# cpockrandt/PhyloCSFpp

Measured on NVIDIA B200. Metric: MAF columns/sec (6 frames, coding+noncoding ECM), higher is better.
Workload: dtype tf32x3/f32

## Files before the change

phylocsfpp_b200/csrc/model_prep.hpp:

```cpp
#pragma once

#include <cmath>
#include <cstdint>
#include <cstring>
#include <string>
#include <vector>

namespace pcsf {

constexpr int NS = 64;

constexpr int SMALL_TREE_MAX_LEAVES = 128;
constexpr int BLS_MAX_WORDS = 8;

struct LeafSet {
    uint64_t w[BLS_MAX_WORDS] = {};
    LeafSet operator|(const LeafSet &o) const { LeafSet r; for (int i = 0; i < BLS_MAX_WORDS; ++i) r.w[i] = w[i] | o.w[i]; return r; }
    LeafSet operator&(const LeafSet &o) const { LeafSet r; for (int i = 0; i < BLS_MAX_WORDS; ++i) r.w[i] = w[i] & o.w[i]; return r; }
    LeafSet operator~() const { LeafSet r; for (int i = 0; i < BLS_MAX_WORDS; ++i) r.w[i] = ~w[i]; return r; }
    bool any() const { uint64_t x = 0; for (int i = 0; i < BLS_MAX_WORDS; ++i) x |= w[i]; return x != 0; }
    int count() const { int c = 0; for (int i = 0; i < BLS_MAX_WORDS; ++i) c += __builtin_popcountll(w[i]); return c; }
    int first() const { for (int i = 0; i < BLS_MAX_WORDS; ++i) if (w[i]) return 64 * i + __builtin_ctzll(w[i]); return -1; }
    void set(int l) { w[l >> 6] |= 1ull << (l & 63); }
    static LeafSet all(int nl) { LeafSet r; for (int l = 0; l < nl; ++l) r.set(l); return r; }
    uint64_t bits(int shift, int nbits) const {
        const int i = shift >> 6, o = shift & 63;
        uint64_t v = w[i] >> o;
        if (o && i + 1 < BLS_MAX_WORDS) v |= w[i + 1] << (64 - o);
        return v & ((1ull << nbits) - 1);
    }
};

enum : int32_t { OP_GATHER_SET = 1, OP_GATHER_MUL = 2, OP_PUSH = 3, OP_POP_MUL = 4, OP_GEMM = 5, OP_END = 6 };
inline int32_t mk_op(int code, int arg) { return (code << 16) | (arg & 0xffff); }

struct BlsNode {
    double bl;
    LeafSet self;
    LeafSet left;
    int32_t is_leaf;
};

struct BlsInner {
    double bl;
    double left_bl, right_bl;
    LeafSet self, left;
    int32_t flags;
    int32_t tab_off;
};
inline int bls_table_shift(int32_t flags) { return ((flags >> 8) & 0xff) | ((flags >> 16) & 0xff00); }
inline int32_t bls_table_flags(int shift, int nbits) { return 4 | ((shift & 0xff) << 8) | (nbits << 16) | ((shift >> 8) << 24); }

template <int NW>
struct BlsInnerDev {
    double bl;
    double left_bl, right_bl;
    uint64_t self[NW], left[NW];
    int32_t flags;
    int32_t tab_off;
};
template <int NW>
inline std::vector<BlsInnerDev<NW>> bls_device_program(const std::vector<BlsInner> &prog) {
    std::vector<BlsInnerDev<NW>> out(prog.size());
    for (size_t k = 0; k < prog.size(); ++k) {
        const BlsInner &e = prog[k];
        BlsInnerDev<NW> &d = out[k];
        d.bl = e.bl; d.left_bl = e.left_bl; d.right_bl = e.right_bl;
        for (int i = 0; i < NW; ++i) { d.self[i] = e.self.w[i]; d.left[i] = e.left.w[i]; }
        d.flags = e.flags; d.tab_off = e.tab_off;
    }
    return out;
}

struct EcmHost {
    double lambda[NS], SR[NS * NS], SRinv[NS * NS], pi[NS], logpi[NS];
    std::vector<double> P;
    std::vector<double> pstream;
    std::vector<double> leafPT;
    std::vector<float> pstream_tc5;
    std::vector<double> cherry_P;
};

struct Tc5Src {
    uint32_t row_base;
    uint8_t l1, l2;
    uint8_t cherry;
    uint8_t pad;
};

struct ModelHost {
    int nl = 0, n = 0;
    std::vector<int16_t> child1, child2;
    std::vector<float> bl;
    std::vector<double> bl64;
    EcmHost ecm[2];
    std::vector<int32_t> program;
    std::vector<int> gemm_edges;
    int max_stack = 0;
    std::vector<uint32_t> tc5_steps;
    std::vector<int> tc5_edges;
    std::vector<int> tc5_leaf_order;
    std::vector<int> tc5_cherries;
    std::vector<uint16_t> tc5_cherry_leaves;
    std::vector<Tc5Src> tc5_srcs;
    uint32_t tc5_rows = 0;
    uint32_t tc5_start = 0;
    int tc5_max_stack = 0;
    std::vector<BlsNode> bls_prog;
    std::vector<BlsInner> bls_inner;
    std::vector<BlsInner> bls_short;
    std::vector<double> bls_tables;
    int bls_short_depth = 0;
    int bls_depth = 0;
    double bls_all = 0.0;
};

inline void build_q(const double *S, const double *f, double *Q) {
    double scale = 0.0;
    for (int i = 0; i < NS; ++i) {
        double rowsum = 0.0;
        for (int j = 0; j < NS; ++j) {
            const double v = S[i * NS + j] * f[j];
            Q[i * NS + j] = v;
            rowsum -= v;
        }
        Q[i * NS + i] = rowsum;
        scale -= rowsum * f[i];
    }
    for (int i = 0; i < NS * NS; ++i) Q[i] /= scale;
}

inline void jacobi64(std::vector<double> &A, std::vector<double> &V, double *w) {
    for (int i = 0; i < NS; ++i)
        for (int j = 0; j < NS; ++j) V[i * NS + j] = (i == j);
    for (int sweep = 0; sweep < 128; ++sweep) {
        double off = 0.0;
        for (int p = 0; p < NS; ++p)
            for (int q = p + 1; q < NS; ++q) off += A[p * NS + q] * A[p * NS + q];
        if (off < 1e-300) break;
        for (int p = 0; p + 1 < NS; ++p)
            for (int q = p + 1; q < NS; ++q) {
                const double apq = A[p * NS + q];
                if (std::fabs(apq) < 1e-310) continue;
                const double theta = (A[q * NS + q] - A[p * NS + p]) / (2.0 * apq);
                const double t = std::copysign(1.0, theta) / (std::fabs(theta) + std::sqrt(theta * theta + 1.0));
                const double c = 1.0 / std::sqrt(t * t + 1.0), s = t * c;
                for (int k = 0; k < NS; ++k) {
                    const double x = A[k * NS + p], y = A[k * NS + q];
                    A[k * NS + p] = c * x - s * y;
                    A[k * NS + q] = s * x + c * y;
                }
                for (int k = 0; k < NS; ++k) {
                    const double x = A[p * NS + k], y = A[q * NS + k];
                    A[p * NS + k] = c * x - s * y;
                    A[q * NS + k] = s * x + c * y;
                }
                for (int k = 0; k < NS; ++k) {
                    const double x = V[k * NS + p], y = V[k * NS + q];
                    V[k * NS + p] = c * x - s * y;
                    V[k * NS + q] = s * x + c * y;
                }
            }
    }
    for (int i = 0; i < NS; ++i) w[i] = A[i * NS + i];
}

inline bool eigen_and_prior(const double *Q, const double *f, EcmHost &e, std::string &err) {
    double sq[NS];
    for (int i = 0; i < NS; ++i) {
        if (!(f[i] > 0.0)) { err = "codon frequencies must be strictly positive"; return false; }
        sq[i] = std::sqrt(f[i]);
    }
    std::vector<double> A(NS * NS), U(NS * NS);
    for (int i = 0; i < NS; ++i)
        for (int j = 0; j < NS; ++j) A[i * NS + j] = sq[i] * Q[i * NS + j] / sq[j];
    for (int i = 0; i < NS; ++i)
        for (int j = i + 1; j < NS; ++j) A[i * NS + j] = A[j * NS + i] = 0.5 * (A[i * NS + j] + A[j * NS + i]);
    jacobi64(A, U, e.lambda);
    for (int i = 0; i < NS; ++i)
        for (int k = 0; k < NS; ++k) {
            e.SR[i * NS + k] = U[i * NS + k] / sq[i];
            e.SRinv[k * NS + i] = U[i * NS + k] * sq[i];
        }
    int kmin = 0;
    double best = std::fabs(e.lambda[0]);
    for (int k = 1; k < NS; ++k)
        if (std::fabs(e.lambda[k]) < best) { best = std::fabs(e.lambda[k]); kmin = k; }
    double mass = 0.0;
    for (int j = 0; j < NS; ++j) mass += e.SRinv[kmin * NS + j];
    for (int j = 0; j < NS; ++j) {
        e.pi[j] = e.SRinv[kmin * NS + j] / mass;
        e.logpi[j] = std::log(e.pi[j]);
    }
    return true;
}

inline double branch_time(float bl, double rho) { return (double)(float)((double)bl * rho); }

inline int pmatrix(const EcmHost &e, double t, double *P) {
    double ex[NS];
    std::vector<double> B(NS * NS);
    for (int k = 0; k < NS; ++k) ex[k] = std::exp(e.lambda[k] * t);
    for (int k = 0; k < NS; ++k)
        for (int j = 0; j < NS; ++j) B[k * NS + j] = e.SRinv[k * NS + j] * ex[k];
    for (int i = 0; i < NS; ++i) {
        double *row = P + i * NS;
        for (int j = 0; j < NS; ++j) row[j] = 0.0;
        for (int k = 0; k < NS; ++k) {
            const double a = e.SR[i * NS + k];
            for (int j = 0; j < NS; ++j) row[j] += a * B[k * NS + j];
        }
    }
    for (int i = 0; i < NS; ++i) {
        double total = 0.0, diag = 1.0;
        for (int j = 0; j < NS; ++j) {
            const double cell = P[i * NS + j];
            total += cell;
            if (cell < 0.0) {
                if (std::fabs(cell) > 1e-6) return 1;
                P[i * NS + j] = 0.0;
            }
            if (i != j) diag -= P[i * NS + j];
        }
        if (std::fabs(total - 1.0) > 1e-6) return 2;
        P[i * NS + i] = diag;
    }
    return 0;
}

inline void to_fragment_order(const double *P, double *tile) {
    for (int ks = 0; ks < 16; ++ks)
        for (int ntp = 0; ntp < 4; ++ntp)
            for (int lane = 0; lane < 32; ++lane)
                for (int e = 0; e < 2; ++e) {
                    const int a = 8 * (2 * ntp + e) + lane / 4;
                    const int b = 8 * (ks / 2) + 2 * (lane % 4) + (ks % 2);
                    tile[((ks * 4 + ntp) * 32 + lane) * 2 + e] = P[a * NS + b];
                }
}

// ... 384 lines not shown
```

phylocsfpp_b200/csrc/pcsf_capi.cu:

```cuda
#include "../../include/phylocsf_b200.h"

#include <cuda_runtime.h>

#include <algorithm>
#include <cmath>
#include <cstdio>
#include <cstdlib>
#include <cstring>
#include <limits>
#include <string>
#include <vector>

#include "kernels.cuh"
#include "mle.cuh"
#include "omega.cuh"
#include "prune_tc5.cuh"
#include "regions.cuh"
#include <nvtx3/nvToolsExt.h>

using namespace pcsf;

static thread_local std::string g_err;
static pcsf_status fail(pcsf_status st, const std::string &msg) { g_err = msg; return st; }

// ... 4 lines not shown
            return fail(PCSF_ERR_CUDA, std::string(#call) + ": " + cudaGetErrorString(e_));        \
    } while (0)

struct DevBuf {
    void *p = nullptr;
    size_t cap = 0;
    cudaError_t reserve(size_t bytes) {
        if (bytes <= cap) return cudaSuccess;
        if (p) cudaFree(p);
        p = nullptr; cap = 0;
        size_t want = bytes + bytes / 4;
        want = (want + ((size_t)2 << 20) - 1) & ~(((size_t)2 << 20) - 1);
        cudaError_t e = cudaMalloc(&p, want);
        if (e != cudaSuccess) { cudaGetLastError(); want = bytes; e = cudaMalloc(&p, want); }
        if (e == cudaSuccess) cap = want;
        return e;
    }
    void release() { if (p) cudaFree(p); p = nullptr; cap = 0; }
    template <class T> T *as() const { return reinterpret_cast<T *>(p); }
};

struct NvtxRange {
    explicit NvtxRange(const char *name) { nvtxRangePushA(name); }
    ~NvtxRange() { nvtxRangePop(); }
};

struct pcsf_model {
    int device = 0;
    int sm_count = 148;
    cudaStream_t own_stream = nullptr;
    cudaStream_t copy_stream = nullptr;
    cudaEvent_t ev_chunk = nullptr;
    double *h_plus = nullptr, *h_minus = nullptr, *h_bls = nullptr;
    uint32_t *h_pat = nullptr;
    const uint8_t *h_seqs = nullptr;
    int64_t h_ld = 0;
    cudaStream_t h2d_stream = nullptr;
    std::vector<cudaEvent_t> ev_h2d;
    ModelHost host;
    double *d_pstream[2] = {nullptr, nullptr}, *d_leafPT[2] = {nullptr, nullptr};
    double *d_pi[2] = {nullptr, nullptr}, *d_logpi[2] = {nullptr, nullptr};
    double *d_eig[2] = {nullptr, nullptr};
    float *d_pstream_tc5[2] = {nullptr, nullptr};
    float *d_rowtab_tc5[2] = {nullptr, nullptr};
    Tc5Src *d_tc5_srcs = nullptr;
    uint32_t *d_tc5_steps = nullptr;
    float *d_tc5_scratch = nullptr;
    size_t prune_tc5_smem = 0;
    int tc5_nstage = 2, tc5_nids = 1;
    MleStats msa_stats;
    uint8_t *h_msa = nullptr;
    size_t h_msa_cap = 0;
    DevBuf tc5_ids;
    int32_t *d_program = nullptr;
    void *d_bls_prog = nullptr;
    double *d_bls_tables = nullptr;
    float *d_bl = nullptr;
    int32_t *d_gemm_edges = nullptr;
    DevBuf codes, klo, khi, slot, flag, uniq, pidx, table, bsums, logz, anc, io_in, io_out, perwin, mle;
    DevBuf rg_units, rg_regions, rg_win;
    std::vector<pcsf_region> regions;
    int *d_bad = nullptr;
    uint32_t *d_nuniq = nullptr;
    int64_t chunk_cols = (int64_t)1 << 21;
    bool timing = false;
    uint32_t stagger_ns = 1000;
    pcsf_tracks_stats last{};
    int64_t last_nwin = 0;
    int launches = 0;
    int last_chunks = 0;
    int64_t codes_ld = 0;
    size_t prune_smem = 0;
    int prune_nwarp = 8;
    cudaEvent_t ev[8] = {};
};

static const int MAX_CHUNKS = 4096;

extern "C" const char *pcsf_last_error(void) { return g_err.c_str(); }
extern "C" int pcsf_abi_version(void) { return PCSF_ABI_VERSION; }

static pcsf_status upload(const void *src, size_t bytes, void **dst) {
    CK(cudaMalloc(dst, bytes ? bytes : 16));
    if (bytes) CK(cudaMemcpy(*dst, src, bytes, cudaMemcpyHostToDevice));
    return PCSF_OK;
}

extern "C" pcsf_status pcsf_model_create(const pcsf_model_desc *d, int device, pcsf_model **out) {
    if (!d || !out || d->nl < 2 || !d->child1 || !d->child2 || !d->branch_len || !d->branch_len_f64 || !d->ecm_c ||
        !d->freq_c || !d->ecm_nc || !d->freq_nc)
        return fail(PCSF_ERR_INVALID, "pcsf_model_create: null argument or fewer than 2 leaves");
    if (d->nl > PCSF_MAX_LEAVES)
        return fail(PCSF_ERR_UNSUPPORTED, "tree of " + std::to_string(d->nl) + " leaves: at most " + std::to_string(PCSF_MAX_LEAVES) +
                                              " leaves (PCSF_MAX_LEAVES) are supported");
    pcsf_model *m = new pcsf_model;
    struct Guard {
        pcsf_model *m;
        ~Guard() { if (m) pcsf_model_destroy(m); }
    } guard{m};
    const double *S[2] = {d->ecm_c, d->ecm_nc}, *f[2] = {d->freq_c, d->freq_nc};
    const std::string err = prepare_model(m->host, d->nl, d->child1, d->child2, d->branch_len, d->branch_len_f64, S, f);
    if (!err.empty()) {
        return fail(err.find("substition_matrix") != std::string::npos ? PCSF_ERR_NUMERIC : PCSF_ERR_INVALID, err);
    }
    int ndev = 0;
    if (cudaGetDeviceCount(&ndev) != cudaSuccess || ndev == 0 || device < 0 || device >= ndev) {
        guard.m = nullptr;
        delete m;
        return fail(PCSF_ERR_CUDA, "no CUDA device available (this library has no CPU fallback)");
    }
    m->device = device;
    if (const char *e = getenv("PCSF_STAGGER_NS")) m->stagger_ns = (uint32_t)atoi(e);
    CK(cudaSetDevice(device));
    CK(cudaDeviceGetAttribute(&m->sm_count, cudaDevAttrMultiProcessorCount, device));
    {
        uint8_t lut[256];
        memset(lut, 255, sizeof lut);
        lut['A'] = lut['a'] = 0; lut['C'] = lut['c'] = 1; lut['G'] = lut['g'] = 2; lut['T'] = lut['t'] = 3;
        lut['.'] = lut['-'] = lut['N'] = lut['n'] = 4;
        CK(cudaMemcpyToSymbol(c_dna_lut, lut, sizeof lut));
    }
    pcsf_status st;
    for (int w = 0; w < 2; ++w) {
        const EcmHost &e = m->host.ecm[w];
        if ((st = upload(e.pstream.data(), e.pstream.size() * 8, (void **)&m->d_pstream[w]))) return st;
        if ((st = upload(e.leafPT.data(), e.leafPT.size() * 8, (void **)&m->d_leafPT[w]))) return st;
        if ((st = upload(e.pstream_tc5.data(), e.pstream_tc5.size() * 4, (void **)&m->d_pstream_tc5[w]))) return st;
        if ((st = upload(e.pi, 64 * 8, (void **)&m->d_pi[w]))) return st;
        if ((st = upload(e.logpi, 64 * 8, (void **)&m->d_logpi[w]))) return st;
        std::vector<double> eig(64 + 2 * 4096);
        memcpy(eig.data(), e.lambda, 64 * 8);
        memcpy(eig.data() + 64, e.SR, 4096 * 8);
        memcpy(eig.data() + 64 + 4096, e.SRinv, 4096 * 8);
        if ((st = upload(eig.data(), eig.size() * 8, (void **)&m->d_eig[w]))) return st;
    }
    if ((st = upload(m->host.program.data(), m->host.program.size() * 4, (void **)&m->d_program))) return st;
    if (m->host.nl <= SMALL_TREE_MAX_LEAVES) {
        if ((st = upload(m->host.tc5_steps.data(), m->host.tc5_steps.size() * 4, (void **)&m->d_tc5_steps))) return st;
        CK(cudaMalloc(&m->d_tc5_scratch, (size_t)m->sm_count * 2 * std::max(1, m->host.tc5_max_stack) * T5_STACK_ENTRY_FLOATS * 4));
        const int ns = (int)m->host.tc5_srcs.size();
        if ((st = upload(m->host.tc5_srcs.data(), (size_t)ns * sizeof(Tc5Src), (void **)&m->d_tc5_srcs))) return st;
        for (int w = 0; w < 2; ++w) {
            double *d_cp = nullptr;
            if ((st = upload(m->host.ecm[w].cherry_P.data(), m->host.ecm[w].cherry_P.size() * 8, (void **)&d_cp))) return st;
            cudaError_t e = cudaMalloc(&m->d_rowtab_tc5[w], (size_t)m->host.tc5_rows * 64 * 4);
            if (e == cudaSuccess) {
                k_build_rows<<<dim3(65, ns), 64>>>(m->d_tc5_srcs, d_cp, m->d_leafPT[w], m->d_rowtab_tc5[w]);
                e = cudaGetLastError();
                if (e == cudaSuccess) e = cudaDeviceSynchronize();
            }
            cudaFree(d_cp);
            CK(e);
        }
        prune_tc5_pick_stages(m->host.nl, (int)m->host.tc5_steps.size(), (int)m->host.tc5_srcs.size(), &m->tc5_nstage, &m->tc5_nids);
        if (const char *e = getenv("PCSF_TC5_NSTAGE")) m->tc5_nstage = std::max(2, std::min(m->tc5_nstage, atoi(e)));
        if (const char *e = getenv("PCSF_TC5_NIDS")) m->tc5_nids = std::max(1, std::min(m->tc5_nids, atoi(e)));
        m->prune_tc5_smem = prune_tc5_smem_bytes(m->host.nl, (int)m->host.tc5_steps.size(), (int)m->host.tc5_srcs.size(), m->tc5_nstage, m->tc5_nids);
        if (m->prune_tc5_smem <= 227 * 1024)
            CK(cudaFuncSetAttribute(k_prune_tc5, cudaFuncAttributeMaxDynamicSharedMemorySize, (int)m->prune_tc5_smem));
        const std::vector<BlsInnerDev<2>> prog = bls_device_program<2>(m->host.bls_short);
        if ((st = upload(prog.data(), prog.size() * sizeof(prog[0]), &m->d_bls_prog))) return st;
    } else {
        const std::vector<BlsInnerDev<8>> prog = bls_device_program<8>(m->host.bls_short);
        if ((st = upload(prog.data(), prog.size() * sizeof(prog[0]), &m->d_bls_prog))) return st;
    }
    if ((st = upload(m->host.bls_tables.data(), std::max<size_t>(m->host.bls_tables.size(), 1) * sizeof(double), (void **)&m->d_bls_tables))) return st;
    if ((st = upload(m->host.bl.data(), m->host.bl.size() * 4, (void **)&m->d_bl))) return st;
    {
        std::vector<int32_t> ge(m->host.gemm_edges.begin(), m->host.gemm_edges.end());
        if ((st = upload(ge.data(), ge.size() * 4, (void **)&m->d_gemm_edges))) return st;
    }
    CK(cudaMalloc(&m->d_bad, sizeof(int)));
    CK(cudaMemset(m->d_bad, 0, sizeof(int)));
    if (!getenv("PCSF_LEGACY_STREAM")) {
        CK(cudaStreamCreateWithFlags(&m->own_stream, cudaStreamNonBlocking));
        CK(cudaStreamCreateWithFlags(&m->copy_stream, cudaStreamNonBlocking));
        CK(cudaStreamCreateWithFlags(&m->h2d_stream, cudaStreamNonBlocking));
        CK(cudaEventCreateWithFlags(&m->ev_chunk, cudaEventDisableTiming));
    }
    CK(cudaMalloc(&m->d_nuniq, sizeof(uint32_t) * MAX_CHUNKS));
    for (auto &e : m->ev) CK(cudaEventCreate(&e));
    m->prune_nwarp = PR_MAX_NWARP;
    if (const char *e = getenv("PCSF_PRUNE_NWARP")) m->prune_nwarp = std::max(1, std::min(PR_MAX_NWARP, atoi(e)));
    while (m->prune_nwarp > 4 &&
           prune_smem_bytes(m->host.nl, (int)m->host.program.size(), m->host.max_stack, m->prune_nwarp) > 227 * 1024)
        m->prune_nwarp -= 4;
    m->prune_smem = prune_smem_bytes(m->host.nl, (int)m->host.program.size(), m->host.max_stack, m->prune_nwarp);
    if (m->prune_smem > 227 * 1024) {
        return fail(PCSF_ERR_UNSUPPORTED, "tree needs more shared memory than one SM has (stack depth " +
                                              std::to_string(m->host.max_stack) + ")");
    }
    CK(cudaFuncSetAttribute(prune_kernel<false>(m->host.nl), cudaFuncAttributeMaxDynamicSharedMemorySize, (int)m->prune_smem));
    CK(cudaFuncSetAttribute(prune_kernel<true>(m->host.nl), cudaFuncAttributeMaxDynamicSharedMemorySize, (int)m->prune_smem));
    CK(cudaFuncSetAttribute(m->host.nl <= SMALL_TREE_MAX_LEAVES ? (const void *)k_bls<2> : (const void *)k_bls<8>,
                            cudaFuncAttributeMaxDynamicSharedMemorySize, std::max(1, m->host.bls_short_depth) * BLS_THREADS * BLS_COLS * 8));
    guard.m = nullptr;
    *out = m;
    return PCSF_OK;
}

extern "C" void pcsf_model_destroy(pcsf_model *m) {
    if (!m) return;
    cudaSetDevice(m->device);
    for (int w = 0; w < 2; ++w) {
        cudaFree(m->d_pstream[w]); cudaFree(m->d_leafPT[w]); cudaFree(m->d_rowtab_tc5[w]); cudaFree(m->d_pstream_tc5[w]); cudaFree(m->d_pi[w]); cudaFree(m->d_logpi[w]);
        cudaFree(m->d_eig[w]);
    }
    cudaFree(m->d_program); cudaFree(m->d_bls_prog); cudaFree(m->d_bls_tables); cudaFree(m->d_bl); cudaFree(m->d_gemm_edges);
    cudaFree(m->d_bad); cudaFree(m->d_nuniq); cudaFree(m->d_tc5_steps); cudaFree(m->d_tc5_scratch); cudaFree(m->d_tc5_srcs);
    if (m->h_msa) cudaFreeHost(m->h_msa);
    if (m->own_stream) cudaStreamDestroy(m->own_stream);
    if (m->copy_stream) cudaStreamDestroy(m->copy_stream);
    if (m->h2d_stream) cudaStreamDestroy(m->h2d_stream);
    for (cudaEvent_t e : m->ev_h2d) cudaEventDestroy(e);
    if (m->ev_chunk) cudaEventDestroy(m->ev_chunk);
    DevBuf *bufs[] = {&m->codes, &m->klo, &m->khi, &m->slot, &m->flag, &m->uniq, &m->pidx, &m->table,
                      &m->bsums, &m->logz, &m->anc, &m->io_in, &m->io_out, &m->perwin, &m->mle, &m->tc5_ids,
                      &m->rg_units, &m->rg_regions, &m->rg_win};
    for (DevBuf *b : bufs) b->release();
    for (auto &e : m->ev) if (e) cudaEventDestroy(e);
    delete m;
}

extern "C" pcsf_status pcsf_score_msa_stats(const pcsf_model *m, pcsf_msa_stats *stats) {
    if (!m || !stats) return fail(PCSF_ERR_INVALID, "pcsf_score_msa_stats: null argument");
    const MleStats &s = m->msa_stats;
    *stats = pcsf_msa_stats{s.alignments, s.evaluations, s.rounds, s.slots, s.ms_step, s.ms_plan, s.ms_expm, s.ms_prune};
    return PCSF_OK;
}

extern "C" pcsf_status pcsf_model_get(const pcsf_model *m, int which, double *lambda, double *pi, double *P) {
    if (!m || which < 0 || which > 1) return fail(PCSF_ERR_INVALID, "pcsf_model_get: bad argument");
    const EcmHost &e = m->host.ecm[which];
    if (lambda) memcpy(lambda, e.lambda, 64 * 8);
    if (pi) memcpy(pi, e.pi, 64 * 8);
    if (P) memcpy(P, e.P.data(), e.P.size() * 8);
    return PCSF_OK;
}

extern "C" pcsf_status pcsf_set_chunk_columns(pcsf_model *m, int64_t columns) {
    if (!m || columns < 0) return fail(PCSF_ERR_INVALID, "pcsf_set_chunk_columns: bad argument");
    if (columns == 0) columns = (int64_t)1 << 21;
    if (columns > ((int64_t)1 << 23)) columns = (int64_t)1 << 23;
    m->chunk_cols = columns;
    return PCSF_OK;
}

extern "C" pcsf_status pcsf_set_timing(pcsf_model *m, int enabled) {
    if (!m) return fail(PCSF_ERR_INVALID, "null model");
    m->timing = enabled != 0;
    return PCSF_OK;
}

static inline uint32_t next_pow2(uint64_t x) {
    uint64_t p = 1;
    while (p < x) p <<= 1;
    return (uint32_t)p;
}

static pcsf_status dedup_and_prune(pcsf_model *m, const WinSpace &ws, uint32_t nwin, bool dedup, bool want_anc, int prec ,
                                   uint32_t *d_nuniq_slot, uint32_t *d_pattern_out, int64_t out_base,
                                   cudaStream_t st, float *ms_hash, float *ms_dedup, float *ms_prune) {
    NvtxRange nvtx_("pcsf: keys + dedup + prune");
    const int TB = 256;
    const uint32_t nblk = (nwin + TB - 1) / TB;
    CK(m->uniq.reserve((size_t)nwin * 4));
    CK(m->pidx.reserve((size_t)nwin * 4));
    CK(m->logz.reserve((size_t)nwin * 16));
    if (want_anc) CK(m->anc.reserve((size_t)nwin * 16));
    if (m->timing) CK(cudaEventRecord(m->ev[0], st));
    if (dedup) {
        CK(m->klo.reserve((size_t)nwin * 8));
        CK(m->khi.reserve((size_t)nwin * 8));
        if (ws.mode == 0) {
            const int64_t ncols = nwin / 2;
            m->launches++;
            if ((ws.c0 & 3) == 0 && (ws.ld & 3) == 0 && (reinterpret_cast<uintptr_t>(ws.codes) & 3) == 0) {
                const int64_t nthr = (ncols + 3) / 4;
                k_keys_tracks<<<(unsigned)((nthr + TB - 1) / TB), TB, 0, st>>>(ws, ncols, m->klo.as<ulonglong2>(), m->khi.as<ulonglong2>());
            } else {
                k_keys_tracks_unaligned<<<(unsigned)((ncols + TB - 1) / TB), TB, 0, st>>>(ws, ncols, m->klo.as<ulonglong2>(), m->khi.as<ulonglong2>());
            }
        } else {
            m->launches++; k_keys_list<<<nblk, TB, 0, st>>>(ws, nwin, m->klo.as<uint64_t>(), m->khi.as<uint64_t>());
        }
        CK(cudaGetLastError());
        if (m->timing) CK(cudaEventRecord(m->ev[1], st));
        const uint32_t T = next_pow2((uint64_t)nwin * 2 < 1024 ? 1024 : (uint64_t)nwin * 2);
        const uint32_t nsb = (nwin + SCAN_BLOCK - 1) / SCAN_BLOCK;
        CK(m->table.reserve((size_t)T * 4));
        CK(m->slot.reserve((size_t)nwin * 4));
        CK(m->flag.reserve((size_t)nwin * 4));
        CK(m->bsums.reserve((size_t)(nsb + 1) * 4));
        CK(cudaMemsetAsync(m->table.p, 0xFF, (size_t)T * 4, st));
        m->launches += 5; k_insert<<<nblk, TB, 0, st>>>(ws, m->klo.as<uint64_t>(), m->khi.as<uint64_t>(), nwin, m->table.as<uint32_t>(), T - 1,
                                      m->slot.as<uint32_t>());
        k_resolve<<<nblk, TB, 0, st>>>(nwin, m->slot.as<uint32_t>(), m->table.as<uint32_t>(), m->flag.as<uint32_t>());
        k_scan_blocks<<<nsb, SCAN_THREADS, 0, st>>>(m->flag.as<uint32_t>(), nwin, m->bsums.as<uint32_t>());
        k_scan_sums<<<1, 1024, 0, st>>>(m->bsums.as<uint32_t>(), nsb, d_nuniq_slot);
        k_finalize<<<nblk, TB, 0, st>>>(nwin, m->slot.as<uint32_t>(), m->flag.as<uint32_t>(), m->bsums.as<uint32_t>(),
                                        m->uniq.as<uint32_t>(), m->pidx.as<uint32_t>(), d_pattern_out, out_base);
        CK(cudaGetLastError());
    } else {
        if (m->timing) CK(cudaEventRecord(m->ev[1], st));
        m->launches++; k_identity<<<nblk, TB, 0, st>>>(nwin, m->uniq.as<uint32_t>(), m->pidx.as<uint32_t>(), d_nuniq_slot, d_pattern_out,
                                        out_base);
// ... 578 lines not shown
```

phylocsfpp_b200/csrc/prune_tc5.cuh:

```cuda
#pragma once

#include "kernels.cuh"
#include "tc5.cuh"

namespace pcsf {

constexpr int T5_MAX_NSTAGE = 3;
constexpr int T5_TILE_BYTES = 32768;
constexpr int T5_THREADS = 512;
constexpr int T5_NPROD = 6;
constexpr int T5_STACK_ENTRY_FLOATS = 64 * 128 + 128;
constexpr int T5_ROW_PITCH = 256;
constexpr int T5_ROW_STAGE_BYTES = 128 * T5_ROW_PITCH;

struct PruneTc5Args {
    const uint32_t *n_unique;
    const uint32_t *steps;
    int nl, n_steps, max_stack;
    int n_src;
    int nstage;
    int nids;
    const uint8_t *ids;
    const float *pstream[2];
    const float *rowtab[2];
    const Tc5Src *srcs;
    const double *pi[2];
    double *logz[2];
    float *scratch;
};

__host__ __device__ inline size_t prune_tc5_smem_bytes(int nl, int n_steps, int n_src, int nstage, int nids) {
    size_t b = (size_t)nstage * T5_TILE_BYTES;
    b += (size_t)2 * 2 * T5_ROW_STAGE_BYTES;
    b += (size_t)T5_NPROD * 256;
    b += (size_t)nids * 2 * nl * 128;
    b += (size_t)(((n_steps + 1) * 4 + 15) / 16) * 16;
    b += (size_t)(n_src + 1) * sizeof(Tc5Src);
    b += 2 * 64 * 8;
    b += 32 * 8;
    return b;
}
inline void prune_tc5_pick_stages(int nl, int n_steps, int n_src, int *nstage, int *nids) {
    *nstage = 2; *nids = 1;
    if (prune_tc5_smem_bytes(nl, n_steps, n_src, 2, 2) <= 227 * 1024) *nids = 2;
    if (prune_tc5_smem_bytes(nl, n_steps, n_src, 3, *nids) <= 227 * 1024) *nstage = 3;
}

__global__ void __launch_bounds__(128) k_tc5_ids(const WinSpace ws, const uint32_t *__restrict__ uniq, const uint32_t *__restrict__ n_unique_p,
                                                 uint8_t *__restrict__ ids) {
    const uint32_t n_unique = *n_unique_p;
    const uint32_t npairs = (n_unique + 255) / 256;
    for (uint32_t pair = blockIdx.x; pair < npairs; pair += gridDim.x) {
        const uint32_t u0 = pair * 256 + 2 * threadIdx.x, u1 = u0 + 1;
        const uint32_t lw0 = uniq[u0 < n_unique ? u0 : n_unique - 1], lw1 = uniq[u1 < n_unique ? u1 : n_unique - 1];
        uint8_t *out = ids + (size_t)pair * 2 * ws.nl * 128 + (size_t)(threadIdx.x >> 6) * ws.nl * 128 + ((2 * threadIdx.x) & 127);
        if (ws.mode == 0 && (lw0 & 1) == 0 && lw1 == lw0 + 1) {
            const uint8_t *p = ws.codes + ws.c0 + (lw0 >> 1);
            for (int s0 = 0; s0 < ws.nl; s0 += 16) {
                uint32_t v[16][3];
#pragma unroll
                for (int k = 0; k < 16; ++k) {
                    const uint8_t *q = p + (int64_t)(s0 + k < ws.nl ? s0 + k : s0) * ws.ld;
                    v[k][0] = __ldg(q); v[k][1] = __ldg(q + 1); v[k][2] = __ldg(q + 2);
                }
#pragma unroll
                for (int k = 0; k < 16; ++k)
                    if (s0 + k < ws.nl)
                        *reinterpret_cast<uint16_t *>(out + (size_t)(s0 + k) * 128) =
                            (uint16_t)(codon_plus(v[k][0], v[k][1], v[k][2]) | (codon_minus(v[k][0], v[k][1], v[k][2]) << 8));
            }
            continue;
        }
#pragma unroll
        for (int h = 0; h < 2; ++h) {
            const uint32_t lw = h ? lw1 : lw0;
            uint32_t strand;
            const int64_t o = win_column(ws, lw, &strand);
            const uint8_t *p = ws.codes + o;
            for (int s0 = 0; s0 < ws.nl; s0 += 16) {
                uint32_t v[16][3];
#pragma unroll
                for (int k = 0; k < 16; ++k) {
                    const uint8_t *q = p + (int64_t)(s0 + k < ws.nl ? s0 + k : s0) * ws.ld;
                    v[k][0] = __ldg(q); v[k][1] = __ldg(q + 1); v[k][2] = __ldg(q + 2);
                }
#pragma unroll
                for (int k = 0; k < 16; ++k)
                    if (s0 + k < ws.nl)
                        out[(size_t)(s0 + k) * 128 + h] = (uint8_t)(strand ? codon_minus(v[k][0], v[k][1], v[k][2]) : codon_plus(v[k][0], v[k][1], v[k][2]));
            }
        }
    }
}

__global__ void __launch_bounds__(64) k_build_rows(const Tc5Src *__restrict__ srcs, const double *__restrict__ cherry_P,
                                                   const double *__restrict__ leafPT, float *__restrict__ tab) {
    __shared__ double u[64];
    __shared__ double v[65][64];
    const Tc5Src d = srcs[blockIdx.y];
    const int x = blockIdx.x, a = threadIdx.x;
    if (d.l2 == 0xff) {
        tab[((size_t)d.row_base + x) * 64 + a] = x < 64 ? (float)leafPT[((size_t)d.l1 * 65 + x) * 64 + a] : 1.0f;
        return;
    }
    u[a] = x < 64 ? leafPT[((size_t)d.l1 * 65 + x) * 64 + a] : 1.0;
    for (int y = 0; y < 65; ++y) v[y][a] = y < 64 ? leafPT[((size_t)d.l2 * 65 + y) * 64 + a] : 1.0;
    __syncthreads();
    double pa[64];
#pragma unroll
    for (int b = 0; b < 64; ++b) pa[b] = cherry_P[(size_t)d.cherry * 4096 + a * 64 + b] * u[b];
    float *out = tab + ((size_t)d.row_base + (size_t)x * 65) * 64 + a;
    for (int y = 0; y < 65; ++y) {
        double s = 0.0;
#pragma unroll
        for (int b = 0; b < 64; ++b) s += pa[b] * v[y][b];
        out[(size_t)y * 64] = (float)s;
    }
}

__device__ __forceinline__ void cp_async_16(uint32_t dst_smem, const void *src) {
    asm volatile("cp.async.cg.shared.global [%0], [%1], 16;" ::"r"(dst_smem), "l"(src) : "memory");
}
__device__ __forceinline__ void cp_async_16_ca(uint32_t dst_smem, const void *src) {
    asm volatile("cp.async.ca.shared.global [%0], [%1], 16;" ::"r"(dst_smem), "l"(src) : "memory");
}
#ifndef PCSF_TC5_ROWS_CA
#define PCSF_TC5_ROWS_CA 2
#endif
__device__ __forceinline__ void cp_async_commit() { asm volatile("cp.async.commit_group;" ::: "memory"); }
template <int N> __device__ __forceinline__ void cp_async_wait() { asm volatile("cp.async.wait_group %0;" ::"n"(N) : "memory"); }

__global__ void __launch_bounds__(T5_THREADS, 1) k_prune_tc5(const PruneTc5Args a) {
    extern __shared__ __align__(1024) unsigned char smem[];
    unsigned char *sp_ = smem;
    const uint32_t T5_NSTAGE = a.nstage;
    unsigned char *stage_buf = sp_; sp_ += (size_t)T5_NSTAGE * T5_TILE_BYTES;
    unsigned char *row_buf = sp_; sp_ += (size_t)2 * 2 * T5_ROW_STAGE_BYTES;
    uint32_t *row_xchg = reinterpret_cast<uint32_t *>(sp_); sp_ += (size_t)T5_NPROD * 256;
    uint8_t *ids = sp_; sp_ += (size_t)a.nids * 2 * a.nl * 128;
    uint32_t *steps = reinterpret_cast<uint32_t *>(sp_); sp_ += (size_t)(((a.n_steps + 1) * 4 + 15) / 16) * 16;
    Tc5Src *srcs = reinterpret_cast<Tc5Src *>(sp_); sp_ += (size_t)(a.n_src + 1) * sizeof(Tc5Src);
    double *s_pi = reinterpret_cast<double *>(sp_); sp_ += 2 * 64 * 8;
    uint64_t *full = reinterpret_cast<uint64_t *>(sp_);
    uint64_t *empty = full + T5_MAX_NSTAGE;
    uint64_t *a_ready = empty + T5_MAX_NSTAGE;
    uint64_t *d_ready = a_ready + 4;
    uint64_t *row_full = d_ready + 2;
    uint64_t *row_empty = row_full + 4;
    uint64_t *ids_full = row_empty + 4;
    uint64_t *ids_empty = ids_full + 2;
    uint32_t *tmem_base_slot = reinterpret_cast<uint32_t *>(ids_empty + 2);

    const int tid = threadIdx.x, warp = tid >> 5, lane = tid & 31;
#ifdef PCSF_TC5_TRACE
    __shared__ long long trace[3][64][4];
    __shared__ long long ptrace[T5_NPROD][56][3];
    __shared__ unsigned short pjob[T5_NPROD][56];
#define T5_TRACE(who, s, i) do { if (blockIdx.x == 0 && first_seq && (s) < 64) trace[who][s][i] = clock64(); } while (0)
#else
#define T5_TRACE(who, s, i) do { } while (0)
#endif
    if (tid == 0) {
        for (int s = 0; s < T5_MAX_NSTAGE; ++s) { mbar_init(full + s, 1); mbar_init(empty + s, 1); }
        for (int c = 0; c < 2; ++c) { for (int k = 0; k < 2; ++k) mbar_init(a_ready + 2 * c + k, 128); mbar_init(d_ready + c, 1); }
        for (int i = 0; i < 4; ++i) { mbar_init(row_full + i, 128); mbar_init(row_empty + i, 128); }
        for (int i = 0; i < 2; ++i) { mbar_init(ids_full + i, 1); mbar_init(ids_empty + i, T5_NPROD); }
        asm volatile("fence.mbarrier_init.release.cluster;" ::: "memory");
    }
    if (warp == 8) { tc5::tmem_alloc(tmem_base_slot, 512); tc5::tmem_relinquish(); }
    for (int i = tid; i < a.n_steps; i += blockDim.x) steps[i] = a.steps[i];
    for (int i = tid; i < a.n_src; i += blockDim.x) srcs[i] = a.srcs[i];
    for (int i = tid; i < 128; i += blockDim.x) s_pi[i] = (i >> 6 ? a.pi[1] : a.pi[0])[i & 63];
    tc5::fence_before_sync();
    __syncthreads();
    tc5::fence_after_sync();
    const uint32_t tmem = *tmem_base_slot;

    const uint32_t n_unique = *a.n_unique;
    const uint32_t npairs = (n_unique + 255) / 256;
    const int n_src2 = 2 * a.n_src;

    if (warp >= 8) {
        asm volatile("setmaxnreg.dec.sync.aligned.u32 40;");
        if (warp == 9) {
            if (lane == 0) {
                uint32_t use = 0;
                for (uint32_t pair = blockIdx.x; pair < npairs; pair += gridDim.x)
                    for (int m = 0; m < 2; ++m)
                        for (int s = 0; s < a.n_steps; ++s, ++use) {
                            const uint32_t st = use % T5_NSTAGE;
                            mbar_wait(empty + st, ((use / T5_NSTAGE) & 1) ^ 1);
                            mbar_arrive_expect_tx(full + st, T5_TILE_BYTES);
                            tma_bulk_g2s(stage_buf + (size_t)st * T5_TILE_BYTES, (m ? a.pstream[1] : a.pstream[0]) + (size_t)s * 8192, T5_TILE_BYTES, full + st);
                        }
            }
        } else if (warp == 8) {
            const uint32_t idesc = tc5::idesc_tf32(128, 128), idesc_hi = tc5::idesc_tf32(128, 64);
            uint32_t use = 0;
            for (uint32_t pair = blockIdx.x; pair < npairs; pair += gridDim.x)
                for (int m = 0; m < 2; ++m)
                    for (int s = 0; s < a.n_steps; ++s, ++use) {
                        const uint32_t st = use % T5_NSTAGE;
#ifdef PCSF_TC5_TRACE
                        const bool first_seq = pair == blockIdx.x + 4 * gridDim.x && m == 0 && lane == 0;
#endif
                        mbar_wait(full + st, (use / T5_NSTAGE) & 1);
                        const uint32_t sb = tc5::smem_addr(stage_buf + (size_t)st * T5_TILE_BYTES);
                        for (int c = 0; c < 2; ++c) {
                            const uint32_t ta = tmem + c * 256 + (use & 1) * 128, td = tmem + c * 256 + ((use & 1) ^ 1) * 128;
#pragma unroll
                            for (int k = 0; k < 2; ++k) {
                                mbar_wait(a_ready + 2 * c + k, use & 1);
                                if (k == 0) T5_TRACE(2, s, 2 * c);
                                tc5::fence_after_sync();
                                if (tc5::elect_one()) {
#pragma unroll
                                    for (int j = 4 * k; j < 4 * k + 4; ++j) {
                                        const uint64_t bd = tc5::smem_desc(sb + j * 4096, 128, 256);
                                        tc5::mma_tf32_ts(td, ta + 8 * j, bd, idesc, j > 0);
                                        tc5::mma_tf32_ts(td, ta + 64 + 8 * j, bd, idesc_hi, 1);
                                    }
                                    if (k == 1) {
                                        tc5::commit(d_ready + c);
                                        if (c == 1) tc5::commit(empty + st);
                                    }
                                }
                                __syncwarp();
                            }
                            __syncwarp();
                            T5_TRACE(2, s, 2 * c + 1);
                        }
                    }
        } else {
            const int pw = warp - 10;
            uint32_t *xchg = row_xchg + pw * 64;
            const uint32_t row_s = tc5::smem_addr(row_buf);
            const int jobs_per_pair = n_src2 * 8;
            const int half = lane >> 4, ch = lane & 15;
            const size_t ids_slot_bytes = (size_t)2 * a.nl * 128;
            uint32_t it = 0;
            uint32_t J = pw;
            const uint32_t my_pairs = npairs > blockIdx.x ? (npairs - blockIdx.x + gridDim.x - 1) / gridDim.x : 0;
            auto load_ids = [&](uint32_t k) {
                const uint32_t slot = k % a.nids, round = k / a.nids;
                mbar_wait_sleepy(ids_empty + slot, (round & 1) ^ 1);
                mbar_arrive_expect_tx(ids_full + slot, (uint32_t)ids_slot_bytes);
                tma_bulk_g2s(ids + slot * ids_slot_bytes, a.ids + ((size_t)blockIdx.x + (size_t)k * gridDim.x) * ids_slot_bytes,
                             (uint32_t)ids_slot_bytes, ids_full + slot);
            };
            if (pw == 0 && lane == 0)
                for (uint32_t k = 0; k < (uint32_t)a.nids - 1 && k < my_pairs; ++k) load_ids(k);
            for (; it < my_pairs; ++it) {
                if (pw == 0 && lane == 0 && it + a.nids - 1 < my_pairs) load_ids(it + a.nids - 1);
                __syncwarp();
                const uint32_t slot = it % a.nids;
                mbar_wait_sleepy(ids_full + slot, (it / a.nids) & 1);
                const uint8_t *pids = ids + slot * ids_slot_bytes;
                const uint32_t jend = (it + 1) * (uint32_t)jobs_per_pair;
                for (; J < jend; J += T5_NPROD) {
                    const uint32_t j = J - it * (uint32_t)jobs_per_pair;
                    const uint32_t q = j & 3, c = (j >> 2) & 1, g = j >> 3;
                    const uint32_t G = it * (uint32_t)n_src2 + g;
                    const int m = g >= (uint32_t)a.n_src ? 1 : 0;
                    const Tc5Src d = srcs[g - m * a.n_src];
                    const uint8_t *wid = pids + (size_t)c * a.nl * 128 + q * 32 + lane;
                    const uint32_t x = wid[(uint32_t)d.l1 * 128];
#if defined(PCSF_TC5_EXP) && PCSF_TC5_EXP == 2
                    const uint32_t myrow = d.row_base + (x & 0u) + q * 32 + lane;
#else
                    const uint32_t myrow = d.row_base + (d.l2 == 0xff ? x : x * 65u + wid[(uint32_t)d.l2 * 128]);
#endif
                    uint32_t *xb = xchg + (((J / T5_NPROD) & 1u) << 5);
                    xb[(lane & 1) * 16 + (lane >> 1)] = myrow;
                    __syncwarp();
                    const uint32_t b = c * 2 + (G & 1);
#ifdef PCSF_TC5_TRACE
                    const uint32_t pj = (J - it * (uint32_t)jobs_per_pair) / T5_NPROD;
                    const bool ptr_on = blockIdx.x == 0 && it == 4 && pj < 56 && lane == 0;
                    if (ptr_on) { ptrace[pw][pj][0] = clock64(); pjob[pw][pj] = (unsigned short)j; }
#endif
                    mbar_wait(row_empty + b, ((G >> 1) & 1) ^ 1);
#ifdef PCSF_TC5_TRACE
                    if (ptr_on) ptrace[pw][pj][1] = clock64();
#endif
                    const float *tab = (m ? a.rowtab[1] : a.rowtab[0]) + ch * 4;
                    const uint32_t dst = row_s + b * T5_ROW_STAGE_BYTES + q * 32 * 256;
                    const bool use_l1 = PCSF_TC5_ROWS_CA == 1 || (PCSF_TC5_ROWS_CA == 2 && d.l2 == 0xff);
#if defined(PCSF_TC5_EXP) && PCSF_TC5_EXP == 1
                    mbar_arrive(row_full + b);
                    (void)tab; (void)dst; (void)use_l1;
                    continue;
#endif
#pragma unroll
                    for (int k = 0; k < 4; ++k) {
                        const uint4 v = reinterpret_cast<const uint4 *>(xb + half * 16)[k];
                        const float *s0 = tab + (size_t)v.x * 64, *s1 = tab + (size_t)v.y * 64, *s2 = tab + (size_t)v.z * 64, *s3 = tab + (size_t)v.w * 64;
                        const int r0 = 2 * (4 * k) + half, r1 = r0 + 2, r2 = r0 + 4, r3 = r0 + 6;
                        const uint32_t d0 = dst + r0 * 256 + (((ch & 8) | ((ch ^ r0) & 7)) << 4), d1 = dst + r1 * 256 + (((ch & 8) | ((ch ^ r1) & 7)) << 4),
                                       d2 = dst + r2 * 256 + (((ch & 8) | ((ch ^ r2) & 7)) << 4), d3 = dst + r3 * 256 + (((ch & 8) | ((ch ^ r3) & 7)) << 4);
                        if (use_l1) { cp_async_16_ca(d0, s0); cp_async_16_ca(d1, s1); cp_async_16_ca(d2, s2); cp_async_16_ca(d3, s3); }
                        else { cp_async_16(d0, s0); cp_async_16(d1, s1); cp_async_16(d2, s2); cp_async_16(d3, s3); }
                    }
                    asm volatile("cp.async.mbarrier.arrive.noinc.shared::cta.b64 [%0];" ::"r"(tc5::smem_addr(row_full + b)) : "memory");
#ifdef PCSF_TC5_TRACE
                    if (ptr_on) ptrace[pw][pj][2] = clock64();
#endif
                }
                __syncwarp();
                if (lane == 0) { tc5::fence_proxy_async_smem(); mbar_arrive(ids_empty + slot); }
            }
        }
    } else {
        asm volatile("setmaxnreg.inc.sync.aligned.u32 216;");
        const int c = warp >> 2, t = tid & 127;
        const uint32_t lane_base = tmem + ((uint32_t)((warp & 3) * 32) << 16) + c * 256;
        float *stk = a.scratch + ((size_t)blockIdx.x * 2 + c) * (size_t)(a.max_stack > 0 ? a.max_stack : 1) * T5_STACK_ENTRY_FLOATS;
        uint32_t use = 0;
        uint32_t taken = 0;
        const unsigned char *rstage = row_buf + (size_t)c * 2 * T5_ROW_STAGE_BYTES + (size_t)t * T5_ROW_PITCH;
        auto take_row = [&](float (&L)[64], bool mul) {
            const uint32_t b = taken & 1;
            mbar_wait(row_full + c * 2 + b, (taken >> 1) & 1);
            const float4 *row = reinterpret_cast<const float4 *>(rstage + b * T5_ROW_STAGE_BYTES);
#pragma unroll
            for (int j = 0; j < 16; ++j) {
                const float4 v = row[(j & 8) | ((j ^ t) & 7)];
                if (mul) { L[4 * j] *= v.x; L[4 * j + 1] *= v.y; L[4 * j + 2] *= v.z; L[4 * j + 3] *= v.w; }
                else { L[4 * j] = v.x; L[4 * j + 1] = v.y; L[4 * j + 2] = v.z; L[4 * j + 3] = v.w; }
            }
            mbar_arrive(row_empty + c * 2 + b);
            ++taken;
        };

#ifdef PCSF_TC5_TRACE
        long long t_seq = 0, t_pro = 0, t_begin = clock64();
#endif
        for (uint32_t pair = blockIdx.x; pair < npairs; pair += gridDim.x) {
            const uint32_t u = pair * 256 + c * 128 + t;
            for (int m = 0; m < 2; ++m) {
                float R[64];
                int E = 0, sp = 0;
#ifdef PCSF_TC5_TRACE
                long long tt1 = clock64();
#endif
                take_row(R, false);
                take_row(R, true);
#ifdef PCSF_TC5_TRACE
                long long tt2 = clock64();
                t_pro += tt2 - tt1;
#endif
                float amax_prev = 0.f;
                auto normalise = [&](float (&V)[64], float &vmax) {
                    float m4[4] = {0.f, 0.f, 0.f, 0.f};
#pragma unroll
                    for (int i = 0; i < 64; i += 8) {
#pragma unroll
                        for (int k = 0; k < 4; ++k) m4[k] = fmaxf(m4[k], fmaxf(V[i + 2 * k], V[i + 2 * k + 1]));
                    }
                    const float mx = fmaxf(fmaxf(m4[0], m4[1]), fmaxf(m4[2], m4[3]));
                    const int e = mx > 0.f ? (int)((__float_as_uint(mx) >> 23) & 0xff) - 127 : 0;
                    const float sc = __uint_as_float((uint32_t)(127 - e) << 23);
                    const float2 sc2 = make_float2(sc, sc);
#pragma unroll
                    for (int i = 0; i < 64; i += 2) {
                        const float2 r = __fmul2_rn(make_float2(V[i], V[i + 1]), sc2);
                        V[i] = r.x; V[i + 1] = r.y;
                    }
                    vmax = mx * sc;
                    return e;
                };
                auto store_A = [&](const float (&V)[64], uint32_t areg) {
#pragma unroll
                    for (int h = 0; h < 4; ++h) {
                        uint32_t hi[16], lo[16];
#pragma unroll
                        for (int i = 0; i < 16; i += 2) {
                            hi[i] = __float_as_uint(V[16 * h + i]) & 0xffffe000u;
                            hi[i + 1] = __float_as_uint(V[16 * h + i + 1]) & 0xffffe000u;
                            const float2 l = __fadd2_rn(make_float2(V[16 * h + i], V[16 * h + i + 1]),
                                                        make_float2(-__uint_as_float(hi[i]), -__uint_as_float(hi[i + 1])));
                            lo[i] = __float_as_uint(l.x);
                            lo[i + 1] = __float_as_uint(l.y);
                        }
                        if (h == 2) {
                            tc5::wait_st();
                            tc5::fence_before_sync();
                            mbar_arrive(a_ready + 2 * c);
                        }
                        tc5::st16(areg + 16 * h, hi);
                        tc5::st16(areg + 64 + 16 * h, lo);
                    }
                    tc5::wait_st();
                    tc5::fence_before_sync();
                    mbar_arrive(a_ready + 2 * c + 1);
                };
                if (a.n_steps > 0) {
                    E += normalise(R, amax_prev);
                    store_A(R, lane_base + (use & 1) * 128);
                }

                for (int s = 0; s < a.n_steps; ++s, ++use) {
                    const uint32_t step = steps[s];
                    const uint32_t post = (step >> 16) & 3u;
#ifdef PCSF_TC5_TRACE
                    const bool first_seq = pair == blockIdx.x + 4 * gridDim.x && m == 0 && (t == 0);
#endif
                    T5_TRACE(c, s, 0);
                    float L[64];
                    int Epop = 0;
                    float amax_start = 0.f;
                    if (post == T5_MUL) {
                        take_row(L, false);
                    } else if (post == T5_PUSH_START) {
                        take_row(L, false);
                        take_row(L, true);
                        Epop = normalise(L, amax_start);
                    } else {
                        --sp;
                        const float4 *e4 = reinterpret_cast<const float4 *>(stk + (size_t)sp * T5_STACK_ENTRY_FLOATS);
#pragma unroll
                        for (int j = 0; j < 16; ++j) {
                            const float4 v = __ldcg(e4 + j * 128 + t);
                            L[4 * j] = v.x; L[4 * j + 1] = v.y; L[4 * j + 2] = v.z; L[4 * j + 3] = v.w;
                        }
                        Epop = __ldcg(reinterpret_cast<const int *>(stk + (size_t)sp * T5_STACK_ENTRY_FLOATS + 8192) + t);
                    }
                    uint32_t dreg = lane_base + ((use & 1) ^ 1) * 128;
                    asm volatile("" : "+r"(dreg));
                    T5_TRACE(c, s, 1);
                    mbar_wait(d_ready + c, use & 1);
                    T5_TRACE(c, s, 2);
                    tc5::fence_after_sync();
                    const int e = amax_prev > 0.f ? (int)((__float_as_uint(amax_prev) >> 23) & 0xff) - 127 : 0;
                    const float sc = __uint_as_float((uint32_t)(127 - e) << 23);
                    const float2 sc2 = make_float2(sc, sc);
                    E += e;
                    if (post == T5_PUSH_START) {
                        float4 *e4 = reinterpret_cast<float4 *>(stk + (size_t)sp * T5_STACK_ENTRY_FLOATS);
#pragma unroll
                        for (int hh = 0; hh < 2; ++hh) {
                            uint32_t x0[32], y0[32];
                            tc5::ld32(dreg + 32 * hh, x0);
                            tc5::ld32(dreg + 64 + 32 * hh, y0);
                            tc5::wait_ld();
#pragma unroll
                            for (int i = 0; i < 32; i += 4) {
                                const float2 v0 = __fmul2_rn(__fadd2_rn(make_float2(__uint_as_float(x0[i]), __uint_as_float(x0[i + 1])),
                                                                        make_float2(__uint_as_float(y0[i]), __uint_as_float(y0[i + 1]))), sc2);
                                const float2 v1 = __fmul2_rn(__fadd2_rn(make_float2(__uint_as_float(x0[i + 2]), __uint_as_float(x0[i + 3])),
                                                                        make_float2(__uint_as_float(y0[i + 2]), __uint_as_float(y0[i + 3]))), sc2);
                                __stcg(e4 + (8 * hh + i / 4) * 128 + t, make_float4(v0.x, v0.y, v1.x, v1.y));
                            }
                        }
                        __stcg(reinterpret_cast<int *>(stk + (size_t)sp * T5_STACK_ENTRY_FLOATS + 8192) + t, E);
                        ++sp;
                        E = Epop;
                        amax_prev = amax_start;
                        store_A(L, dreg);
                    } else if (s + 1 == a.n_steps) {
                        uint32_t x0[32], y0[32], x1[32], y1[32];
                        tc5::ld32(dreg, x0);
                        tc5::ld32(dreg + 64, y0);
                        tc5::ld32(dreg + 32, x1);
                        tc5::ld32(dreg + 96, y1);
                        tc5::wait_ld();
#pragma unroll
                        for (int i = 0; i < 32; i += 2) {
                            float2 v0 = __fmul2_rn(__fadd2_rn(make_float2(__uint_as_float(x0[i]), __uint_as_float(x0[i + 1])),
                                                              make_float2(__uint_as_float(y0[i]), __uint_as_float(y0[i + 1]))), sc2);
                            float2 v1 = __fmul2_rn(__fadd2_rn(make_float2(__uint_as_float(x1[i]), __uint_as_float(x1[i + 1])),
                                                              make_float2(__uint_as_float(y1[i]), __uint_as_float(y1[i + 1]))), sc2);
                            v0 = __fmul2_rn(v0, make_float2(L[i], L[i + 1]));
                            v1 = __fmul2_rn(v1, make_float2(L[32 + i], L[32 + i + 1]));
                            R[i] = v0.x; R[i + 1] = v0.y; R[32 + i] = v1.x; R[32 + i + 1] = v1.y;
                        }
                        E += Epop;
                    } else {
                        E += Epop;
                        float amax = 0.f;
                        float V[64];
                        {
// ... 69 lines not shown
```

Measured before the change: 125.5 million.

## Skip row gathers for all-gap cherry rows that are all ones

```diff
diff --git a/phylocsfpp_b200/csrc/model_prep.hpp b/phylocsfpp_b200/csrc/model_prep.hpp
--- a/phylocsfpp_b200/csrc/model_prep.hpp
+++ b/phylocsfpp_b200/csrc/model_prep.hpp
@@ -85,7 +85,7 @@
     uint32_t row_base;
     uint8_t l1, l2;
     uint8_t cherry;
-    uint8_t pad;
+    uint8_t ones;
 };
 
 struct ModelHost {
diff --git a/phylocsfpp_b200/csrc/pcsf_capi.cu b/phylocsfpp_b200/csrc/pcsf_capi.cu
--- a/phylocsfpp_b200/csrc/pcsf_capi.cu
+++ b/phylocsfpp_b200/csrc/pcsf_capi.cu
@@ -180,6 +180,16 @@
             cudaFree(d_cp);
             CK(e);
         }
+        for (Tc5Src &d : m->host.tc5_srcs) {
+            d.ones = 1;
+            if (d.l2 == 0xff) continue;
+            for (int w = 0; w < 2 && d.ones; ++w) {
+                float row[64];
+                CK(cudaMemcpy(row, m->d_rowtab_tc5[w] + ((size_t)d.row_base + 64 * 65 + 64) * 64, sizeof(row), cudaMemcpyDeviceToHost));
+                for (int a = 0; a < 64; ++a) d.ones &= row[a] == 1.0f;
+            }
+        }
+        CK(cudaMemcpy(m->d_tc5_srcs, m->host.tc5_srcs.data(), (size_t)ns * sizeof(Tc5Src), cudaMemcpyHostToDevice));
         prune_tc5_pick_stages(m->host.nl, (int)m->host.tc5_steps.size(), (int)m->host.tc5_srcs.size(), &m->tc5_nstage, &m->tc5_nids);
         if (const char *e = getenv("PCSF_TC5_NSTAGE")) m->tc5_nstage = std::max(2, std::min(m->tc5_nstage, atoi(e)));
         if (const char *e = getenv("PCSF_TC5_NIDS")) m->tc5_nids = std::max(1, std::min(m->tc5_nids, atoi(e)));
diff --git a/phylocsfpp_b200/csrc/prune_tc5.cuh b/phylocsfpp_b200/csrc/prune_tc5.cuh
--- a/phylocsfpp_b200/csrc/prune_tc5.cuh
+++ b/phylocsfpp_b200/csrc/prune_tc5.cuh
@@ -149,7 +149,8 @@
     uint64_t *row_empty = row_full + 4;
     uint64_t *ids_full = row_empty + 4;
     uint64_t *ids_empty = ids_full + 2;
-    uint32_t *tmem_base_slot = reinterpret_cast<uint32_t *>(ids_empty + 2);
+    uint32_t *row_ones = reinterpret_cast<uint32_t *>(ids_empty + 2);
+    uint32_t *tmem_base_slot = steps + a.n_steps;
 
     const int tid = threadIdx.x, warp = tid >> 5, lane = tid & 31;
 #ifdef PCSF_TC5_TRACE
@@ -163,7 +164,7 @@
     if (tid == 0) {
         for (int s = 0; s < T5_MAX_NSTAGE; ++s) { mbar_init(full + s, 1); mbar_init(empty + s, 1); }
         for (int c = 0; c < 2; ++c) { for (int k = 0; k < 2; ++k) mbar_init(a_ready + 2 * c + k, 128); mbar_init(d_ready + c, 1); }
-        for (int i = 0; i < 4; ++i) { mbar_init(row_full + i, 128); mbar_init(row_empty + i, 128); }
+        for (int i = 0; i < 4; ++i) { mbar_init(row_full + i, 4 * 33); mbar_init(row_empty + i, 128); }
         for (int i = 0; i < 2; ++i) { mbar_init(ids_full + i, 1); mbar_init(ids_empty + i, T5_NPROD); }
         asm volatile("fence.mbarrier_init.release.cluster;" ::: "memory");
     }
@@ -268,8 +269,10 @@
 #if defined(PCSF_TC5_EXP) && PCSF_TC5_EXP == 2
                     const uint32_t myrow = d.row_base + (x & 0u) + q * 32 + lane;
 #else
-                    const uint32_t myrow = d.row_base + (d.l2 == 0xff ? x : x * 65u + wid[(uint32_t)d.l2 * 128]);
-#endif
+                    const uint32_t y = d.l2 == 0xff ? 64u : wid[(uint32_t)d.l2 * 128];
+                    const uint32_t myrow = d.row_base + (d.l2 == 0xff ? x : x * 65u + y);
+#endif
+                    const bool skip = __all_sync(0xffffffffu, d.ones && x == 64u && y == 64u);
                     uint32_t *xb = xchg + (((J / T5_NPROD) & 1u) << 5);
                     xb[(lane & 1) * 16 + (lane >> 1)] = myrow;
                     __syncwarp();
@@ -283,6 +286,7 @@
 #ifdef PCSF_TC5_TRACE
                     if (ptr_on) ptrace[pw][pj][1] = clock64();
 #endif
+                    if (lane == 0) { row_ones[b * 4 + q] = skip; mbar_arrive(row_full + b); }
                     const float *tab = (m ? a.rowtab[1] : a.rowtab[0]) + ch * 4;
                     const uint32_t dst = row_s + b * T5_ROW_STAGE_BYTES + q * 32 * 256;
                     const bool use_l1 = PCSF_TC5_ROWS_CA == 1 || (PCSF_TC5_ROWS_CA == 2 && d.l2 == 0xff);
@@ -293,6 +297,7 @@
 #endif
 #pragma unroll
                     for (int k = 0; k < 4; ++k) {
+                        if (skip) break;
                         const uint4 v = reinterpret_cast<const uint4 *>(xb + half * 16)[k];
                         const float *s0 = tab + (size_t)v.x * 64, *s1 = tab + (size_t)v.y * 64, *s2 = tab + (size_t)v.z * 64, *s3 = tab + (size_t)v.w * 64;
                         const int r0 = 2 * (4 * k) + half, r1 = r0 + 2, r2 = r0 + 4, r3 = r0 + 6;
@@ -321,12 +326,19 @@
         auto take_row = [&](float (&L)[64], bool mul) {
             const uint32_t b = taken & 1;
             mbar_wait(row_full + c * 2 + b, (taken >> 1) & 1);
-            const float4 *row = reinterpret_cast<const float4 *>(rstage + b * T5_ROW_STAGE_BYTES);
-#pragma unroll
-            for (int j = 0; j < 16; ++j) {
-                const float4 v = row[(j & 8) | ((j ^ t) & 7)];
-                if (mul) { L[4 * j] *= v.x; L[4 * j + 1] *= v.y; L[4 * j + 2] *= v.z; L[4 * j + 3] *= v.w; }
-                else { L[4 * j] = v.x; L[4 * j + 1] = v.y; L[4 * j + 2] = v.z; L[4 * j + 3] = v.w; }
+            if (row_ones[(c * 2 + b) * 4 + (t >> 5)]) {
+                if (!mul) {
+#pragma unroll
+                    for (int j = 0; j < 64; ++j) L[j] = 1.0f;
+                }
+            } else {
+                const float4 *row = reinterpret_cast<const float4 *>(rstage + b * T5_ROW_STAGE_BYTES);
+#pragma unroll
+                for (int j = 0; j < 16; ++j) {
+                    const float4 v = row[(j & 8) | ((j ^ t) & 7)];
+                    if (mul) { L[4 * j] *= v.x; L[4 * j + 1] *= v.y; L[4 * j + 2] *= v.z; L[4 * j + 3] *= v.w; }
+                    else { L[4 * j] = v.x; L[4 * j + 1] = v.y; L[4 * j + 2] = v.z; L[4 * j + 3] = v.w; }
+                }
             }
             mbar_arrive(row_empty + c * 2 + b);
             ++taken;
```

After: 126.6 million, median of 6. No clear change (+0.9%).
